# cvg/EMAP

Measured on AMD Instinct MI355X. Metric: ray-samples/sec (UDF MLP + composite), higher is better.
Workload: dtype f16x3 (split-fp16 MFMA, 3 passes, fp32 accumulate)

## Files before the change

### emap_amd/csrc/emap_common.h

```cpp
#pragma once
#include <hip/hip_runtime.h>
#include <stdint.h>
#include <stdio.h>
#include "../../include/emap_hip.h"


namespace emap {
constexpr float F16X3_WS = 8192.0f;
constexpr float F16_LO_SCALE = 2048.0f;

void set_error(const char* fmt, ...);
int check_launch(const char* what);

inline bool attr_needed(uint64_t& mask) {
    int d = 0;
    if (hipGetDevice(&d) != hipSuccess || d < 0 || d > 63) return true;
    if (mask & (1ull << d)) return false;
    mask |= 1ull << d;
    return true;
}
inline int raise_lds_limit(uint64_t& mask, const void* fn, int bytes = 160 * 1024) {
    if (attr_needed(mask) && hipFuncSetAttribute(fn, hipFuncAttributeMaxDynamicSharedMemorySize, bytes) != hipSuccess) {
        set_error("hipFuncSetAttribute(MaxDynamicSharedMemorySize) failed");
        return EMAP_E_LAUNCH;
    }
    return EMAP_OK;
}

constexpr int FRAG_BYTES = 1024;
constexpr int PE_KS = 2;

struct LayerDesc {
    int32_t pe_ks;
    int32_t h_ks;
    int32_t n_pairs;
    int32_t out_dim;
    int32_t in_prev;
    int32_t frag_off;
    int32_t act;
    int32_t pad;
};

struct NetLayout {
    int32_t H, n_lin, skip_l, multires, d0, nparts, udf_type, n_chunks;
    float scale;
    int32_t total_frags;
    int32_t bias_off_bytes, rowscale_off_bytes, frag_off_bytes;
    int32_t is_f16;
    int32_t mx_fwd;
    int32_t mx_bwd;
    int32_t has_rev, t_total_frags, t_frag_off_bytes, wlast_off_bytes;
    int32_t t_off[EMAP_MAX_LIN], tpe_off[EMAP_MAX_LIN];
    int32_t r32_frag_off_bytes, r32_t_frag_off_bytes;
    int32_t sweep_mx, swm_off_bytes, swm_units;
    int32_t wgrad_lo;
    int32_t swm_unit[EMAP_MAX_LIN], swm_t_unit[EMAP_MAX_LIN];
    LayerDesc layer[EMAP_MAX_LIN];
};
constexpr int SWM_UNIT_BYTES = 6656;
__host__ __device__ inline int t_hidden_frags(const NetLayout& L, int l) { return ((L.layer[l].in_prev + 31) / 32) * (L.H / 32) * 2 * L.nparts; }
__host__ __device__ inline int t_pe_frags(const NetLayout& L) { return 2 * (L.H / 32) * 2 * L.nparts; }
__host__ __device__ inline int swm_fwd_units(const NetLayout& L, int l) { return L.layer[l].n_pairs * (L.H / 128); }
__host__ __device__ inline int swm_rev_units(const NetLayout& L, int l) { return ((L.layer[l].in_prev + 31) / 32) * (L.H / 128); }

__host__ __device__ inline bool r32_t_mixed(const NetLayout& L) { return L.mx_bwd && L.is_f16 && L.nparts == 2 && L.H == 256; }
__host__ __device__ inline bool r32_mixed(const NetLayout& L) { return L.mx_fwd && r32_t_mixed(L); }
#define EMAP_PE_HI6_E8M0 125u
#define EMAP_PE_LO6_E8M0 124u
__host__ __device__ inline uint32_t mx6_scale_bits(float m) {
    const float mm = fmaxf(m, 7.8886090522101181e-31f ) * 1.0666667f;
    uint32_t b;
    __builtin_memcpy(&b, &mm, 4);
    return (b & 0x7f800000u) - (2u << 23);
}

int build_layout(const EmapNetConfig* cfg, int prec, NetLayout* L);
inline size_t layout_bytes(const NetLayout& L) {
    const size_t base = (size_t)L.r32_t_frag_off_bytes + (size_t)L.t_total_frags * FRAG_BYTES;
    return L.sweep_mx ? (size_t)L.swm_off_bytes + (size_t)L.swm_units * SWM_UNIT_BYTES : base;
}

int launch_pack(const NetLayout& L, const float* const* g, const float* const* v, const float* const* b,
                void* packed, hipStream_t st);

struct PointSource {
    const float* x;
    const float* rays_o;
// ... 201 lines not shown
```

### emap_amd/csrc/udf_mlp_vjp.inc

```
#pragma once

__device__ __forceinline__ void asm_gload4(uint32_t& dst, int voff, const char* sbase) {
    asm volatile("s_nop 4\n\tglobal_load_dword %0, %1, %2" : "=v"(dst) : "v"(voff), "s"(sbase) : "memory");
}
template <int N>
__device__ __forceinline__ void asm_wait_unit(u32x4& a, u32x4& b, u32x4& c, u32x4& d, u32x2& e, u32x2& f, u32x2& g, u32x2& h, uint32_t& i) {
    asm volatile("s_waitcnt vmcnt(%c9)" : "+v"(a), "+v"(b), "+v"(c), "+v"(d), "+v"(e), "+v"(f), "+v"(g), "+v"(h), "+v"(i) : "i"(N) : "memory");
}


struct VjpArgs {
    MlpArgs m;
    const float* d_udf;
    const float* d_grad;
    char* stash_a;
    char* stash_z;
    char* stash_s;
    const uint32_t* absmax;
    float* ldot;
    VjpLayout V;
    int32_t tile0;
    const char* swm;
    int32_t swm_unit[EMAP_MAX_LIN], swm_t_unit[EMAP_MAX_LIN];
};

template <int H, int MODE, int NW, bool SMX_ = false>
__global__ __launch_bounds__(NW * 64, NW == 8 ? 1 : 2) void udf_mlp_vjp_kernel(const VjpArgs va) {
    using T = typename Prec<MODE>::T;
    using V8 = typename Prec<MODE>::V;
    const MlpArgs& a = va.m;
    constexpr int NPART = Prec<MODE>::NPART;
    constexpr bool SCALED = (NPART == 2);
    constexpr float LO_SCALE = (MODE == EMAP_PREC_F16X3) ? F16_LO_SCALE : 1.0f;
    constexpr int NCT = 4;
    constexpr int NKS = H / 32;
    constexpr int NPAIR = H / 32;
    constexpr int NFR = 2 * NPART;
    constexpr int PD = 2;
    constexpr int PPW = NPAIR / NW;
    constexpr int KQ = NKS / NW;
    static_assert(PPW == 1 && PPW * NW == NPAIR && KQ * NW == NKS && NW >= 4, "waves per workgroup");
    constexpr bool SMX = SMX_ && MODE == EMAP_PREC_F16X3 && H == 256;
    constexpr int NSLAB = vjp_slab_planes(MODE == EMAP_PREC_F16X3, SMX);
    constexpr bool SLABLO = NSLAB > 4;
    typedef uint32_t u32x8 __attribute__((ext_vector_type(8)));

    extern __shared__ __attribute__((aligned(16))) char smem[];
    constexpr int XB = NKS * NCT * NPART * FRAG_BYTES;
    constexpr int PB = PE_KS * NCT * NPART * FRAG_BYTES;
    constexpr bool PP = (NW == 8);
    char* const xb0 = smem;
    char* const xb1 = smem + (PP ? XB : 0);
    char* pebuf = smem + (PP ? 2 : 1) * XB;
    float* red = reinterpret_cast<float*>(PP ? smem + 2 * XB + PB : smem);
    int cur = 0;

    const int tid = threadIdx.x;
    const int lane = tid & 63;
    const int wave = __builtin_amdgcn_readfirstlane(tid >> 6);
    const int g = lane >> 4;
    const int j = lane & 15;
    const int wvoff = lane * 16;
    const char* wbase = uniform_ptr(a.frags);
    const char* tbase = uniform_ptr(a.tfrags);
    const int n_hidden = a.n_lin - 1;
    const char* xr = xb0 + lane * 16;
    const int xm_lane = g * (NCT * NPART * FRAG_BYTES) + FRAG_BYTES;
    const char* xmr = xb0 + xm_lane;
    const char* per = pebuf + lane * 16;
    const int p0 = wave * PPW;
    V8 sel[2];
#pragma unroll
    for (int h = 0; h < 2; ++h)
#pragma unroll
        for (int e = 0; e < 8; ++e) sel[h][e] = ((j >> 2) == g && e == 4 * h + (j & 3)) ? (T)1.0f : (T)0.0f;
    char* const slab = va.stash_s + (size_t)blockIdx.x * ((size_t)va.V.s_slab_kb * 1024);
    const float Kscale = vjp_scale_from(va.absmax);

    clock_stamp(a.clk, 2);
    V8 hd[PD][NFR];
    auto load_head = [&](const char* wb) __attribute__((always_inline)) {
#pragma unroll
        for (int sp = 0; sp < PD; ++sp)
#pragma unroll
            for (int f = 0; f < NFR; ++f) {
                typedef const V8 __attribute__((address_space(1))) * gptr_t;
                hd[sp][f] = *(gptr_t)(uintptr_t)(wb + (sp * NFR + f) * FRAG_BYTES + wvoff);
            }
    };
    u32x2 hd6r[4];
    uint32_t hasc = 0;
    auto load_head_mx = [&](const char* wbh, const char* wm) __attribute__((always_inline)) {
        typedef const V8 __attribute__((address_space(1))) * gptr_t;
        typedef const u32x2 __attribute__((address_space(1))) * g2_t;
        typedef const uint32_t __attribute__((address_space(1))) * g1_t;
#pragma unroll
        for (int sp = 0; sp < PD; ++sp)
#pragma unroll
            for (int t = 0; t < 2; ++t) hd[sp][t] = *(gptr_t)(uintptr_t)(wbh + (sp * NFR + 2 * t) * FRAG_BYTES + wvoff);
#pragma unroll
        for (int t = 0; t < 2; ++t)
#pragma unroll
            for (int pt = 0; pt < 2; ++pt) {
                hd[t][2 + pt] = *(gptr_t)(uintptr_t)(wm + (2 * t + pt) * 1024 + wvoff);
                hd6r[2 * t + pt] = *(g2_t)(uintptr_t)(wm + 4096 + (2 * t + pt) * 512 + lane * 8);
            }
        hasc = *(g1_t)(uintptr_t)(wm + 6144 + lane * 4);
    };
    auto head_after_fwd = [&](int l) __attribute__((always_inline)) {
        int ln = l + 1;
        while (ln < n_hidden && p0 >= a.layer[ln].n_pairs) ++ln;
        const LayerDesc Ln = a.layer[ln < n_hidden ? ln : a.n_lin - 1];
        if constexpr (SMX) {
            if (ln >= n_hidden) return;
            if (!Ln.pe_ks) {
                load_head_mx(wbase + (size_t)(Ln.frag_off + p0 * Ln.h_ks * NFR) * FRAG_BYTES,
                             va.swm + (size_t)(va.swm_unit[ln] + p0 * (NKS / 4)) * SWM_UNIT_BYTES);
                return;
            }
        }
        const int first = (ln < n_hidden) ? p0 * (Ln.pe_ks + Ln.h_ks) : Ln.pe_ks + KQ * wave;
        load_head(wbase + (size_t)(Ln.frag_off + first * NFR) * FRAG_BYTES);
    };
    auto head_after_bwd = [&](int b, int tile) __attribute__((always_inline)) {
        int bn = b - 1;
        while (bn >= 1 && p0 >= a.layer[bn - 1].n_pairs) --bn;
        if (bn >= 1) {
            if constexpr (SMX) load_head_mx(tbase + (size_t)(a.t_off[bn] + p0 * NKS * NFR) * FRAG_BYTES,
                                            va.swm + (size_t)(va.swm_t_unit[bn] + p0 * (NKS / 4)) * SWM_UNIT_BYTES);
            else load_head(tbase + (size_t)(a.t_off[bn] + p0 * NKS * NFR) * FRAG_BYTES);
        }
        else if (tile + (int)gridDim.x < a.n_tiles) head_after_fwd(-1);
    };
    if ((int)blockIdx.x < a.n_tiles) head_after_fwd(-1);
    for (int i = tid * 16; i < (PP ? 2 : 1) * XB; i += NW * 64 * 16) *reinterpret_cast<f32x4*>(smem + i) = f32x4{0.f, 0.f, 0.f, 0.f};
    __syncthreads();
    for (int tile = blockIdx.x; tile < a.n_tiles; tile += gridDim.x) {
        const long long pbase = ((long long)va.tile0 + tile) * VJP_PT;
        char* const sa = va.stash_a + (size_t)tile * ((size_t)va.V.a_tile_kb * 1024);
        char* const sz = va.stash_z + (size_t)tile * ((size_t)va.V.z_tile_kb * 1024);
        constexpr bool LO_STASH = (NPART == 2) && !SMX;
        const bool stash_lo = LO_STASH && va.V.lo_a_delta != 0;
        auto stash_store = [&](char* level_pair, const V8 (&x)[4], int n_rt) __attribute__((always_inline)) {
            const f32x4 z4 = {0.f, 0.f, 0.f, 0.f};
#pragma unroll
            for (int h = 0; h < 2; ++h) {
                if (h < n_rt) {
                    f32x4 d[4];
#pragma unroll
                    for (int ct = 0; ct < 4; ++ct) d[ct] = mfma16(x[ct], sel[h], z4);
#pragma unroll
                    for (int ks = 0; ks < 2; ++ks) {
                        V8 v;
#pragma unroll
                        for (int e = 0; e < 8; ++e) v[e] = (T)d[2 * ks + (e >> 2)][e & 3];
                        *reinterpret_cast<V8*>(level_pair + (h * 2 + ks) * 1024 + lane * 16) = v;
                    }
                }
            }
        };

        if (wave < NCT) {
            const int ct = wave;
            int gq = g;
            asm volatile("" : "+v"(gq));
            float xs[3], vd[3] = {0.f, 0.f, 0.f};
            long long pp = pbase + 16 * (ct & 1) + j;
            const bool valid = pp < a.P;
            if (!valid) pp = a.P - 1;
            load_point(a.src, pp, a.scale, xs);
            if (ct >= 2 && valid) {
                vd[0] = va.d_grad[3 * pp + 0] * Kscale;
                vd[1] = va.d_grad[3 * pp + 1] * Kscale;
                vd[2] = va.d_grad[3 * pp + 2] * Kscale;
            }
            V8 f[PE_KS][NPART];
#pragma unroll
            for (int q = 0; q < 8; ++q) {
                const PeAngle ang = pe_angle(xs, 8 * gq + q, a.multires);
                float v0, v1;
                if (ct < 2) {
                    pe_pair(ang, xs, a.multires, 0, v0, v1);
                } else {
                    const float vc = (ang.c == 0) ? vd[0] : ((ang.c == 1) ? vd[1] : vd[2]);
                    const bool r0 = ang.a == 3 * a.multires, r1 = ang.a == 3 * a.multires + 1;
                    v0 = ang.is_ang ? ang.f * ang.cs * vc : (r0 ? vd[0] : (r1 ? vd[2] : 0.0f));
                    v1 = ang.is_ang ? -ang.f * ang.sn * vc : (r0 ? vd[1] : 0.0f);
                }
                const T h0 = (T)v0, h1 = (T)v1;
                f[q >> 2][0][2 * (q & 3)] = h0;
                f[q >> 2][0][2 * (q & 3) + 1] = h1;
                if constexpr (NPART == 2) {
                    f[q >> 2][1][2 * (q & 3)] = (T)((v0 - (float)h0) * LO_SCALE);
                    f[q >> 2][1][2 * (q & 3) + 1] = (T)((v1 - (float)h1) * LO_SCALE);
                }
            }
#pragma unroll
            for (int sp = 0; sp < PE_KS; ++sp)
#pragma unroll
                for (int pt = 0; pt < NPART; ++pt)
                    *reinterpret_cast<V8*>(pebuf + ((sp * NCT + ct) * NPART + pt) * FRAG_BYTES + lane * 16) = f[sp][pt];
        }
        __syncthreads();
        if (wave >= NW - PE_KS) {
            const int sp = wave - (NW - PE_KS);
            V8 c4[NCT];
#pragma unroll
            for (int ct = 0; ct < NCT; ++ct) c4[ct] = *reinterpret_cast<const V8*>(per + ((sp * NCT + ct) * NPART + 0) * FRAG_BYTES);
            stash_store(sa + (size_t)va.V.a_off[0] * 1024 + (2 * sp) * 2048, c4, 2);
            if constexpr (LO_STASH) {
                if (stash_lo) {
#pragma unroll
                    for (int ct = 0; ct < NCT; ++ct) c4[ct] = *reinterpret_cast<const V8*>(per + ((sp * NCT + ct) * NPART + (NPART - 1)) * FRAG_BYTES);
                    stash_store(sa + va.V.lo_a_delta + (size_t)va.V.a_off[0] * 1024 + (2 * sp) * 2048, c4, 2);
                }
            }
        }

        f32x4 acc[2][NCT];
        f32x4 accx[SCALED ? 2 : 1][NCT];
        V8 o[NCT][NPART];
        const f32x4 zero4 = {0.f, 0.f, 0.f, 0.f};

        auto zval = [&](int t, int ct, int r) __attribute__((always_inline)) -> float {
            if constexpr (SCALED) return fmaf(accx[t][ct][r], 1.0f / LO_SCALE, acc[t][ct][r]);
            else return acc[t][ct][r];
        };

        auto k_run_p = [&](auto ns_c, auto npe_c, auto init_c, auto pre_c, const char* wb, int xs0, int pes0, const float* bp) __attribute__((always_inline)) {
            constexpr int NS = decltype(ns_c)::value;
            constexpr int NPE = decltype(npe_c)::value;
            constexpr bool INIT = decltype(init_c)::value;
            constexpr bool PRE = decltype(pre_c)::value;
            V8 af[PD + 1][NFR];
            auto load_a = [&](auto s_c) __attribute__((always_inline)) {
                constexpr int s = decltype(s_c)::value;
#pragma unroll
                for (int f = 0; f < NFR; ++f) asm_gload16(af[s % (PD + 1)][f], wvoff, wb + (s * NFR + f) * FRAG_BYTES);
            };
            if constexpr (PRE) {
#pragma unroll
                for (int sp = 0; sp < PD; ++sp)
#pragma unroll
                    for (int f = 0; f < NFR; ++f) af[sp][f] = hd[sp][f];
            } else static_for<PD>([&](auto i_c) __attribute__((always_inline)) { if constexpr (decltype(i_c)::value < NS) load_a(i_c); });
            f32x4 i0 = zero4, i1 = zero4;
            if constexpr (INIT) {
                i0 = *reinterpret_cast<const f32x4*>(bp);
                i1 = *reinterpret_cast<const f32x4*>(bp + 16);
            }
            const char* xq = xr + xs0 * (NCT * NPART * FRAG_BYTES);
            const char* pq = per + pes0 * (NCT * NPART * FRAG_BYTES);
            V8 bh[NCT], bl[NCT];
            static_for<NS>([&](auto s_c) __attribute__((always_inline)) {
                constexpr int s = decltype(s_c)::value;
                constexpr int sa_ = s % (PD + 1);
                if constexpr (s == 0 && INIT) asm volatile("" : "+v"(i0), "+v"(i1));
                if constexpr (s + PD < NS) load_a(std::integral_constant<int, s + PD>{});
                constexpr bool is_pe = s < NPE;
                constexpr int sb = is_pe ? s : s - NPE;
#pragma unroll
                for (int ct = 0; ct < NCT; ++ct) {
                    const char* base = is_pe ? pq : xq;
                    bh[ct] = *reinterpret_cast<const V8*>(base + ((sb * NCT + ct) * NPART + 0) * FRAG_BYTES);
                    bl[ct] = *reinterpret_cast<const V8*>(base + ((sb * NCT + ct) * NPART + (NPART - 1)) * FRAG_BYTES);
                }
                {
                    constexpr int younger = ((s + PD < NS) ? PD : (NS - 1 - s)) * NFR;
#pragma unroll
                    for (int f = 0; f < NFR; f += 2) asm_wait_vm<younger>(af[sa_][f], af[sa_][f + 1]);
                }
                if constexpr (s == 0) {
#pragma unroll
                    for (int c2 = 0; c2 < NCT; ++c2) {
                        acc[0][c2] = (c2 < 2) ? i0 : zero4;
                        acc[1][c2] = (c2 < 2) ? i1 : zero4;
                        if constexpr (SCALED) { accx[0][c2] = zero4; accx[1][c2] = zero4; }
                    }
                }
                if constexpr (NPART == 1) {
#pragma unroll
                    for (int ct = 0; ct < NCT; ++ct) {
                        acc[0][ct] = mfma16(af[sa_][0], bh[ct], acc[0][ct]);
                        acc[1][ct] = mfma16(af[sa_][1], bh[ct], acc[1][ct]);
                    }
                } else {
#pragma unroll
                    for (int ct = 0; ct < NCT; ++ct) {
                        if constexpr (SCALED) { accx[0][ct] = mfma16(af[sa_][0], bl[ct], accx[0][ct]); accx[1][ct] = mfma16(af[sa_][2], bl[ct], accx[1][ct]); }
                        else { acc[0][ct] = mfma16(af[sa_][0], bl[ct], acc[0][ct]); acc[1][ct] = mfma16(af[sa_][2], bl[ct], acc[1][ct]); }
                    }
#pragma unroll
                    for (int ct = 0; ct < NCT; ++ct) {
                        acc[0][ct] = mfma16(af[sa_][0], bh[ct], acc[0][ct]);
                        acc[1][ct] = mfma16(af[sa_][2], bh[ct], acc[1][ct]);
                    }
#pragma unroll
// ... 149 lines not shown
                            const auto s02 = __builtin_amdgcn_permlane32_swap(x0, x2, false, false);
                            const auto s13 = __builtin_amdgcn_permlane32_swap(x1, x3, false, false);
                            const auto w01 = __builtin_amdgcn_permlane16_swap(s02[0], s13[0], false, false);
                            const auto w23 = __builtin_amdgcn_permlane16_swap(s02[1], s13[1], false, false);
                            blk[pt][0 * 4 + d] = w01[0]; blk[pt][1 * 4 + d] = w01[1]; blk[pt][2 * 4 + d] = w23[0]; blk[pt][3 * 4 + d] = w23[1];
                        }
                    auto block_max = [&](const u32x16& v) __attribute__((always_inline)) -> float {
                        uint32_t mb = 0;
#pragma unroll
                        for (int q = 0; q < 16; ++q)
                            asm("v_pk_maximum3_f16 %0, %1, %2, %2 neg_lo:[0,0,1] neg_hi:[0,0,1]" : "=v"(mb) : "v"(mb), "v"(v[q]));
                        const h2 m = __builtin_bit_cast(h2, mb);
                        return fmaxf((float)m[0], (float)m[1]);
                    };
                    const uint32_t sbh = mx6_scale_bits(block_max(blk[0])), sbl = mx6_scale_bits(block_max(blk[1]));
                    const u32x6 qh = __builtin_amdgcn_cvt_scalef32_pk32_fp6_f16(__builtin_bit_cast(f16x32, blk[0]), __builtin_bit_cast(float, sbh));
                    const u32x6 ql = __builtin_amdgcn_cvt_scalef32_pk32_fp6_f16(__builtin_bit_cast(f16x32, blk[1]), __builtin_bit_cast(float, sbl));
                    char* const dst = xbuf + ((p0 * NCT + g) * NPART + 1) * FRAG_BYTES;
                    *reinterpret_cast<u32x4*>(dst + j * 16) = u32x4{qh[0], qh[1], qh[2], qh[3]};
                    *reinterpret_cast<u32x4*>(dst + 256 + j * 16) = u32x4{ql[0], ql[1], ql[2], ql[3]};
                    *reinterpret_cast<u32x2*>(dst + 512 + j * 8) = u32x2{qh[4], qh[5]};
                    *reinterpret_cast<u32x2*>(dst + 640 + j * 8) = u32x2{ql[4], ql[5]};
                    *reinterpret_cast<uint32_t*>(dst + 768 + j * 4) = (sbh >> 23) | ((((sbl >> 23) - 11u) & 0xffu) << 8);
                }
            }
            __syncthreads();
            if constexpr (PP) { cur ^= 1; xr = (cur ? xb1 : xb0) + lane * 16; xmr = (cur ? xb1 : xb0) + xm_lane; }
        };
        using yes_t = std::true_type;
        using no_t = std::false_type;
        u32x4 sgv[4];
        auto load_slab = [&](const char* src) __attribute__((always_inline)) {
            const char* sb = uniform_ptr(src);
            static_for<4>([&](auto c_c) __attribute__((always_inline)) {
                constexpr int c = decltype(c_c)::value;
                asm_gload16_sc1<c * 1024>(sgv[c], wvoff, sb);
            });
        };
        auto wait_slab = [&]() __attribute__((always_inline)) {
            asm volatile("s_waitcnt vmcnt(0)" : "+v"(sgv[0]), "+v"(sgv[1]), "+v"(sgv[2]), "+v"(sgv[3]) : : "memory");
        };

        for (int l = 0; l < n_hidden; ++l) {
            const LayerDesc L = a.layer[l];
            const int kind = (L.h_ks == 0) ? KIND_FIRST : (L.pe_ks ? KIND_SKIP : KIND_NORMAL);
            const int p = p0;
            if (p < L.n_pairs) {
                const float* bp = a.bias + l * H + 32 * p + 4 * g;
                const int ns = L.pe_ks + L.h_ks;
                const char* wb = wbase + (size_t)(L.frag_off + p * ns * NFR) * FRAG_BYTES;
                if constexpr (SMX) {
                    const char* wm = va.swm + (size_t)(va.swm_unit[l] + p * (NKS / 4)) * SWM_UNIT_BYTES;
                    if (kind == KIND_NORMAL) k_run_mx(std::integral_constant<int, 1>{}, std::integral_constant<int, NKS / 4>{}, yes_t{}, 0, wb, wm, bp);
                    else if (kind == KIND_SKIP) {
                        k_run_p(std::integral_constant<int, PE_KS>{}, std::integral_constant<int, PE_KS>{}, yes_t{}, yes_t{}, wb, 0, 0, bp);
                        k_run_mx(std::integral_constant<int, 2>{}, std::integral_constant<int, NKS / 4>{}, no_t{}, 0, wb + (size_t)PE_KS * NFR * FRAG_BYTES, wm, bp);
                    } else k_run_p(std::integral_constant<int, PE_KS>{}, std::integral_constant<int, PE_KS>{}, yes_t{}, yes_t{}, wb, 0, 0, bp);
                } else {
                if (kind == KIND_NORMAL) k_run_p(std::integral_constant<int, NKS>{}, std::integral_constant<int, 0>{}, yes_t{}, yes_t{}, wb, 0, 0, bp);
                else if (kind == KIND_SKIP) k_run_p(std::integral_constant<int, PE_KS + NKS>{}, std::integral_constant<int, PE_KS>{}, yes_t{}, yes_t{}, wb, 0, 0, bp);
                else k_run_p(std::integral_constant<int, PE_KS>{}, std::integral_constant<int, PE_KS>{}, yes_t{}, yes_t{}, wb, 0, 0, bp);
                }
                head_after_fwd(l);
                uint32_t bk[SLABLO ? 24 : 16];
                static_for<8>([&](auto q_c) __attribute__((always_inline)) {
                    constexpr int q = decltype(q_c)::value, t = q >> 2, r = q & 3;
                    float a0, s0, a1, s1;
                    softplus_sig_fast(zval(t, 0, r), a0, s0);
                    softplus_sig_fast(zval(t, 1, r), a1, s1);
                    const float t0 = s0 * zval(t, 2, r), t1 = s1 * zval(t, 3, r);
                    put1(0, 4 * t + r, a0);
                    put1(1, 4 * t + r, a1);
                    typedef T T2 __attribute__((ext_vector_type(2)));
                    const T2 ap2 = {put1(2, 4 * t + r, t0), put1(3, 4 * t + r, t1)};
                    bk[2 * q] = __builtin_bit_cast(uint32_t, ap2);
                    bk[2 * q + 1] = __builtin_bit_cast(uint32_t, __builtin_amdgcn_cvt_pknorm_u16(s0, s1));
                    if constexpr (SLABLO) {
                        const T2 lo2 = {(T)((t0 - (float)ap2[0]) * LO_SCALE), (T)((t1 - (float)ap2[1]) * LO_SCALE)};
                        bk[16 + q] = __builtin_bit_cast(uint32_t, lo2);
                    }
                });
                {
                    const V8 xh[4] = {o[0][0], o[1][0], o[2][0], o[3][0]};
                    stash_store(sa + (size_t)va.V.a_off[l + 1] * 1024 + (2 * p) * 2048, xh, 2);
                }
                if constexpr (LO_STASH) {
                    if (stash_lo) {
                        const V8 xl[4] = {o[0][NPART - 1], o[1][NPART - 1], o[2][NPART - 1], o[3][NPART - 1]};
                        stash_store(sa + va.V.lo_a_delta + (size_t)va.V.a_off[l + 1] * 1024 + (2 * p) * 2048, xl, 2);
                    }
                }
                u32x4* dst = reinterpret_cast<u32x4*>(slab + ((size_t)(l * NPAIR + p) * NSLAB) * 1024 + lane * 16);
#pragma unroll
                for (int c = 0; c < NSLAB; ++c) dst[c * 64] = u32x4{bk[4 * c], bk[4 * c + 1], bk[4 * c + 2], bk[4 * c + 3]};
            }
            publish(L.n_pairs);
        }

        float hpart[NCT];
        {
            const LayerDesc L = a.layer[a.n_lin - 1];
            const char* wb = wbase + (size_t)(L.frag_off + (L.pe_ks + KQ * wave) * NFR) * FRAG_BYTES;
            if constexpr (SMX) {
#pragma unroll
                for (int ct = 0; ct < NCT; ++ct) hpart[ct] = 0.f;
                if (wave < NKS / 4) {
                    k_run_mx(std::integral_constant<int, 0>{}, std::integral_constant<int, 1>{}, no_t{}, wave, wbase + (size_t)L.frag_off * FRAG_BYTES,
                             va.swm + (size_t)va.swm_unit[a.n_lin - 1] * SWM_UNIT_BYTES, nullptr);
#pragma unroll
                    for (int ct = 0; ct < NCT; ++ct) hpart[ct] = zval(0, ct, 0);
                }
            } else {
            k_run_p(std::integral_constant<int, KQ>{}, std::integral_constant<int, 0>{}, no_t{}, yes_t{}, wb, KQ * wave, 0, nullptr);
#pragma unroll
            for (int ct = 0; ct < NCT; ++ct) hpart[ct] = zval(0, ct, 0);
            }
            if (L.pe_ks && wave < PE_KS) {
                const char* wp = wbase + (size_t)(L.frag_off + wave * NFR) * FRAG_BYTES;
                k_run(std::integral_constant<int, 1>{}, std::integral_constant<int, 1>{}, no_t{}, wp, 0, wave, nullptr);
#pragma unroll
                for (int ct = 0; ct < NCT; ++ct) hpart[ct] += zval(0, ct, 0);
            }
            head_after_bwd(a.n_lin - 1, tile);
            if constexpr (!PP) __syncthreads();
            if (g == 0) {
#pragma unroll
                for (int ct = 0; ct < NCT; ++ct) red[(wave * NCT + ct) * 16 + j] = hpart[ct];
            }
        }
        __syncthreads();
        float seed[NCT];
        {
            float hs[NCT];
#pragma unroll
            for (int ct = 0; ct < NCT; ++ct) {
                float v = 0.f;
#pragma unroll
                for (int w = 0; w < NW; ++w) v += red[(w * NCT + ct) * 16 + j];
                hs[ct] = v;
            }
            const float b_last = a.bias[(a.n_lin - 1) * H];
            const float inv_scale = 1.0f / a.scale;
            bool bad = false;
#pragma unroll
            for (int c = 0; c < 2; ++c) {
                const long long pp = pbase + 16 * c + j;
                const float h = hs[c] + b_last, hp = hs[c + 2];
                float u1, u2;
                if (a.udf_type == EMAP_UDF_ABS) { u1 = (h > 0.f) ? 1.f : ((h < 0.f) ? -1.f : 0.f); u2 = 0.f; }
                else if (a.udf_type == EMAP_UDF_SQUARE) { u1 = 2.f * h; u2 = 2.f; }
                else { u1 = 1.f; u2 = 0.f; }
                const bool valid = pp < a.P;
                const float du = valid ? va.d_udf[pp] * Kscale : 0.f;
                seed[c] = valid ? fmaf(du * inv_scale, u1, u2 * hp) : 0.f;
                seed[c + 2] = valid ? u1 : 0.f;
                bad |= valid && !(fabsf(h) + fabsf(hp) <= 3.0e38f);
            }
            if (wave == 0 && g == 0) flag_nonfinite(a.err, bad);
            if (wave == 0 && g == 0) {
                float d = seed[0] * hs[0] + seed[1] * hs[1] + seed[2] * hs[2] + seed[3] * hs[3];
#pragma unroll
                for (int off = 8; off > 0; off >>= 1) d += __shfl_xor(d, off);
                if (j == 0) va.ldot[va.tile0 + tile] = d;
            }
        }
        if (wave == 0) {
            V8 xs[4];
#pragma unroll
            for (int ct = 0; ct < NCT; ++ct) {
                const T hi = (T)seed[ct];
#pragma unroll
                for (int e = 0; e < 8; ++e) xs[ct][e] = (T)0.0f;
                xs[ct][0] = (g == 0) ? hi : (T)0.0f;
                xs[ct][1] = (g == 0) ? (T)(seed[ct] - (float)hi) : (T)0.0f;
            }
            stash_store(sz + (size_t)va.V.z_off[a.n_lin - 1] * 1024, xs, 1);
            if constexpr (LO_STASH) {
                if (stash_lo) {
#pragma unroll
                    for (int ct = 0; ct < NCT; ++ct)
#pragma unroll
                        for (int e = 0; e < 8; ++e) xs[ct][e] = (T)0.0f;
                    stash_store(sz + va.V.lo_z_delta + (size_t)va.V.z_off[a.n_lin - 1] * 1024, xs, 1);
                }
            }
        }

        for (int b = a.n_lin - 1; b >= 1; --b) {
            const int lz = b - 1;
            const int p = p0;
            if (p < a.layer[lz].n_pairs) {
                load_slab(slab + ((size_t)(lz * NPAIR + p) * NSLAB) * 1024);
                if (b == a.n_lin - 1) {
                    const f32x4 w0 = *reinterpret_cast<const f32x4*>(a.wlast + 32 * p + 4 * g);
                    const f32x4 w1 = *reinterpret_cast<const f32x4*>(a.wlast + 32 * p + 16 + 4 * g);
#pragma unroll
                    for (int ct = 0; ct < NCT; ++ct) {
                        acc[0][ct] = w0 * seed[ct];
                        acc[1][ct] = w1 * seed[ct];
                        if constexpr (SCALED) { accx[0][ct] = zero4; accx[1][ct] = zero4; }
                    }
                } else {
                    const char* wb = tbase + (size_t)(a.t_off[b] + p * NKS * NFR) * FRAG_BYTES;
                    if constexpr (SMX) k_run_mx(std::integral_constant<int, 0>{}, std::integral_constant<int, NKS / 4>{}, yes_t{}, 0, wb,
                                                va.swm + (size_t)(va.swm_t_unit[b] + p * (NKS / 4)) * SWM_UNIT_BYTES, nullptr);
                    else k_run_p(std::integral_constant<int, NKS>{}, std::integral_constant<int, 0>{}, no_t{}, yes_t{}, wb, 0, 0, nullptr);
                }
                wait_slab();
                u32x4 aplo[2];
                if constexpr (SLABLO) {
                    const char* lp = uniform_ptr(slab + ((size_t)(lz * NPAIR + p) * NSLAB + 4) * 1024);
                    asm_gload16_sc1<0>(aplo[0], wvoff, lp);
                    asm_gload16_sc1<1024>(aplo[1], wvoff, lp);
                    asm volatile("s_waitcnt vmcnt(0)" : "+v"(aplo[0]), "+v"(aplo[1]) : : "memory");
                }
                if (b != a.n_lin - 1) head_after_bwd(b, tile);
                static_for<8>([&](auto q_c) __attribute__((always_inline)) {
                    constexpr int q = decltype(q_c)::value, t = q >> 2, r = q & 3;
                    typedef T T2 __attribute__((ext_vector_type(2)));
                    const uint32_t apk = sgv[q >> 1][2 * (q & 1)], spk = sgv[q >> 1][2 * (q & 1) + 1];
                    const T2 ap2 = __builtin_bit_cast(T2, apk);
                    float ap0 = (float)ap2[0], ap1 = (float)ap2[1];
                    if constexpr (SLABLO) {
                        const uint32_t lok = aplo[q >> 2][q & 3];
                        const T2 lo2 = __builtin_bit_cast(T2, lok);
                        ap0 = fmaf((float)lo2[0], 1.0f / LO_SCALE, ap0);
                        ap1 = fmaf((float)lo2[1], 1.0f / LO_SCALE, ap1);
                    }
                    const float s0 = (float)(spk & 0xffffu) * (1.0f / 65535.0f);
                    const float s1 = (float)(spk >> 16) * (1.0f / 65535.0f);
                    const float av0 = zval(t, 0, r), av1 = zval(t, 1, r), at0 = zval(t, 2, r), at1 = zval(t, 3, r);
                    const float zb0 = fmaf(100.0f * (1.0f - s0) * ap0, at0, s0 * av0);
                    const float zb1 = fmaf(100.0f * (1.0f - s1) * ap1, at1, s1 * av1);
                    put1(0, 4 * t + r, zb0);
                    put1(1, 4 * t + r, zb1);
                    put1(2, 4 * t + r, s0 * at0);
                    put1(3, 4 * t + r, s1 * at1);
                });
                {
                    const V8 xh[4] = {o[0][0], o[1][0], o[2][0], o[3][0]};
                    stash_store(sz + (size_t)va.V.z_off[lz] * 1024 + (2 * p) * 2048, xh, 2);
                }
                if constexpr (LO_STASH) {
                    if (stash_lo) {
                        const V8 xl[4] = {o[0][NPART - 1], o[1][NPART - 1], o[2][NPART - 1], o[3][NPART - 1]};
                        stash_store(sz + va.V.lo_z_delta + (size_t)va.V.z_off[lz] * 1024 + (2 * p) * 2048, xl, 2);
                    }
                }
            }
            if (b > 1) publish(a.layer[lz].n_pairs);
        }
        __syncthreads();
    }
    clock_stamp(a.clk, 3);
}

template <int H, int MODE, int NW, bool SMX_ = false>
static int launch_vjp_sweep_t(const NetLayout& L, const void* packed, const VjpSweep& s, hipStream_t st, int32_t* err) {
    constexpr int NPART = Prec<MODE>::NPART;
    VjpArgs va;
    memset(&va, 0, sizeof(va));
    va.m = fill_mlp_args(L, packed, L.frag_off_bytes, L.t_frag_off_bytes, s.src, s.P, err);
    va.m.n_tiles = s.n_tiles; va.tile0 = s.tile0;
    va.m.clk = prof_clk_here();
    va.d_udf = s.d_udf; va.d_grad = s.d_grad; va.stash_a = s.stash_a; va.stash_z = s.stash_z; va.stash_s = s.stash_s; va.absmax = s.absmax; va.ldot = s.ldot; va.V = *s.V;
    va.swm = static_cast<const char*>(packed) + L.swm_off_bytes;
    for (int l = 0; l < L.n_lin; ++l) { va.swm_unit[l] = L.swm_unit[l]; va.swm_t_unit[l] = L.swm_t_unit[l]; }
    const size_t lds = (NW == 8) ? (size_t)(2 * (H / 32) + PE_KS) * 4 * NPART * FRAG_BYTES + (size_t)NW * 4 * 16 * 4
                                 : (size_t)((H / 32) + PE_KS) * 4 * NPART * FRAG_BYTES;
    auto kern = udf_mlp_vjp_kernel<H, MODE, NW, SMX_>;
    static uint64_t attr_mask = 0;
    const int rc = raise_lds_limit(attr_mask, reinterpret_cast<const void*>(kern));
    if (rc) return rc;
    if (s.n_tiles <= 0) return EMAP_OK;
    hipLaunchKernelGGL(kern, dim3(s.grid < s.n_tiles ? s.grid : s.n_tiles), dim3(NW * 64), lds, st, va);
    return check_launch("udf_mlp_vjp");
}

template <int MODE>
int launch_vjp_sweep_mode(const NetLayout& L, const void* packed, const VjpSweep& s, hipStream_t st, int32_t* err) {
    if constexpr (MODE == EMAP_PREC_F16X3) {
        if (L.H == 256 && L.sweep_mx) return launch_vjp_sweep_t<256, MODE, 8, true>(L, packed, s, st, err);
    }
    if (L.H == 256) return launch_vjp_sweep_t<256, MODE, 8>(L, packed, s, st, err);
    if (L.H == 128) return launch_vjp_sweep_t<128, MODE, 4>(L, packed, s, st, err);
    set_error("no training-backward kernel for d_hidden=%d", L.H);
    return EMAP_E_INVALID;
}
```

### emap_amd/csrc/wgrad.hip

```cpp
#include "emap_common.h"
#include <string.h>

namespace emap {

typedef __bf16 bf16x8 __attribute__((ext_vector_type(8)));
typedef _Float16 f16x8 __attribute__((ext_vector_type(8)));
typedef float f32x4 __attribute__((ext_vector_type(4)));

__device__ __forceinline__ f32x4 mfma16w(const bf16x8& a, const bf16x8& b, const f32x4& c) { return __builtin_amdgcn_mfma_f32_16x16x32_bf16(a, b, c, 0, 0, 0); }
__device__ __forceinline__ f32x4 mfma16w(const f16x8& a, const f16x8& b, const f32x4& c) { return __builtin_amdgcn_mfma_f32_16x16x32_f16(a, b, c, 0, 0, 0); }

__global__ __launch_bounds__(256) void absmax_kernel(const float* du, const float* dg, long long P, uint32_t* out) {
    float mu = 0.f, mg = 0.f;
    for (long long i = (long long)blockIdx.x * 256 + threadIdx.x; i < P; i += (long long)gridDim.x * 256) {
        const float u = fabsf(du[i]);
        const float g = fmaxf(fmaxf(fabsf(dg[3 * i]), fabsf(dg[3 * i + 1])), fabsf(dg[3 * i + 2]));
        mu = (u < 3.0e38f) ? fmaxf(mu, u) : mu;
        mg = (g < 3.0e38f) ? fmaxf(mg, g) : mg;
    }
#pragma unroll
    for (int off = 32; off > 0; off >>= 1) { mu = fmaxf(mu, __shfl_xor(mu, off)); mg = fmaxf(mg, __shfl_xor(mg, off)); }
    if ((threadIdx.x & 63) == 0) {
        atomicMax(out, __builtin_bit_cast(uint32_t, mu));
        atomicMax(out + 1, __builtin_bit_cast(uint32_t, mg));
    }
}

struct WgradArgs {
    const char* stash_a;
    const char* stash_z;
    float* partial;
    int32_t n_tiles, n_jobs, a_tile_kb, z_tile_kb;
    int32_t accumulate;
    float scale;
    int32_t no_bias;
    WgradJob job[WGRAD_MAX_JOBS];
};

template <int CT>
__device__ __forceinline__ void wgrad_store(const WgradArgs& a, const WgradJob& J, int slice, int wave, int lane, f32x4 (&acc)[2][CT], float (&bsum)[2]) {
    float* pb = a.partial + J.part_off + (size_t)slice * 16 * J.a_ct * 256;
#pragma unroll
    for (int i = 0; i < 2; ++i) {
        const int rt = wave + 8 * i;
        if (rt < J.z_rt) {
#pragma unroll
            for (int c = 0; c < CT; ++c) {
                if (c < J.a_ct) {
                    f32x4* dst = reinterpret_cast<f32x4*>(pb + ((size_t)rt * J.a_ct + c) * 256 + lane * 4);
                    *dst = a.accumulate ? (*dst + acc[i][c] * a.scale) : acc[i][c] * a.scale;
                }
            }
        }
    }
    if (J.bias_off >= 0 && !a.no_bias) {
#pragma unroll
        for (int i = 0; i < 2; ++i) {
            float v = bsum[i] * a.scale;
            v += __shfl_xor(v, 16);
            v += __shfl_xor(v, 32);
            const int rt = wave + 8 * i;
            if (rt < J.z_rt && lane < 16) {
                float* dst = a.partial + J.bias_off + (size_t)slice * 256 + rt * 16 + lane;
                *dst = a.accumulate ? (*dst + v) : v;
            }
        }
    }
}

#ifndef EMAP_REDUCE_WAVES
#define EMAP_REDUCE_WAVES 4
#endif
#ifndef EMAP_WGRAD_DEPTH
#define EMAP_WGRAD_DEPTH 3
#endif
constexpr int WGRAD_DEPTH = EMAP_WGRAD_DEPTH;
__device__ __forceinline__ void wg_dma16(unsigned lds_dst, const char* gsrc) {
    unsigned keep;
    asm volatile("s_mov_b32 %0, m0\n\ts_mov_b32 m0, %2\n\ts_nop 0\n\tglobal_load_lds_dwordx4 %1, off\n\ts_mov_b32 m0, %0"
                 : "=&s"(keep) : "v"(gsrc), "s"(lds_dst) : "memory");
}

template <class V8, int NB>
__device__ __forceinline__ void wgrad_lds_run(const WgradArgs& a, const WgradJob& J, int slice, int wave, int lane, char* smem) {
    constexpr int CT = 4 * NB;
    constexpr int NA = (CT + 7) / 8;
    constexpr int NLD = NA + 2;
    constexpr int D = WGRAD_DEPTH, NST = D + 1;
    constexpr int STAGE = (CT + 16) * 1024;
    const int t0 = (int)(((long long)a.n_tiles * slice) / J.n_slices), t1 = (int)(((long long)a.n_tiles * (slice + 1)) / J.n_slices);
    const int nsteps = 2 * (t1 - t0);
    f32x4 acc[2][CT];
#pragma unroll
    for (int i = 0; i < 2; ++i)
#pragma unroll
        for (int c = 0; c < CT; ++c) acc[i][c] = f32x4{0.f, 0.f, 0.f, 0.f};
    float bsum[2] = {0.f, 0.f};
    if (nsteps > 0) {
        const size_t zts = (size_t)a.z_tile_kb * 1024, ats = (size_t)a.a_tile_kb * 1024;
        const char* zsrc = a.stash_z + (size_t)J.z_off * 1024 + lane * 16;
        const char* asrc = a.stash_a + (size_t)J.a_off * 1024 + lane * 16;
        const unsigned lds0 = (unsigned)(size_t)smem;
        int ca[NA], zr[2];
#pragma unroll
        for (int i = 0; i < NA; ++i) ca[i] = 8 * i + ((8 * i + 8 <= CT) ? wave : wave % (CT - 8 * i));
        zr[0] = wave < J.z_rt ? wave : J.z_rt - 1;
        zr[1] = wave + 8 < J.z_rt ? wave + 8 : J.z_rt - 1;
        auto issue = [&](int u) __attribute__((always_inline)) {
            const int uu = u < nsteps ? u : nsteps - 1;
            const int tile = t0 + (uu >> 1), sh = (uu & 1) * 1024;
            const unsigned st = lds0 + (unsigned)(u % NST) * STAGE;
#pragma unroll
            for (int i = 0; i < NA; ++i) {
                const int cs = ca[i] < J.a_ct ? ca[i] : J.a_ct - 1;
                wg_dma16(__builtin_amdgcn_readfirstlane(st + ca[i] * 1024), asrc + (size_t)tile * ats + cs * 2048 + sh);
            }
#pragma unroll
            for (int i = 0; i < 2; ++i)
                wg_dma16(__builtin_amdgcn_readfirstlane(st + (CT + zr[i]) * 1024), zsrc + (size_t)tile * zts + zr[i] * 2048 + sh);
        };
        for (int u = 0; u < D; ++u) issue(u);
        for (int u = 0; u < nsteps; ++u) {
            asm volatile("s_waitcnt vmcnt(%0)" :: "i"(NLD * (D - 1)) : "memory");
            __builtin_amdgcn_s_barrier();
            issue(u + D);
            const char* st = smem + (size_t)(u % NST) * STAGE + lane * 16;
            V8 z[2];
            z[0] = *reinterpret_cast<const V8*>(st + (CT + zr[0]) * 1024);
            z[1] = *reinterpret_cast<const V8*>(st + (CT + zr[1]) * 1024);
            {
                const float m = (u & 1) ? 0.0f : 1.0f;
#pragma unroll
                for (int i = 0; i < 2; ++i)
                    bsum[i] = fmaf(m, (((float)z[i][0] + (float)z[i][1]) + ((float)z[i][2] + (float)z[i][3])) +
                                      (((float)z[i][4] + (float)z[i][5]) + ((float)z[i][6] + (float)z[i][7])), bsum[i]);
            }
#pragma unroll
            for (int c = 0; c < CT; ++c) {
                const V8 af = *reinterpret_cast<const V8*>(st + c * 1024);
                acc[0][c] = mfma16w(z[0], af, acc[0][c]);
                acc[1][c] = mfma16w(z[1], af, acc[1][c]);
            }
        }
        asm volatile("s_waitcnt vmcnt(0)" ::: "memory");
    }
    wgrad_store<CT>(a, J, slice, wave, lane, acc, bsum);
}

#ifdef EMAP_WGRAD_TIMING
static __device__ long long emap_wg_times[1024 * 2];
#endif
template <class V8>
__global__ __launch_bounds__(512, 1) void wgrad_kernel(const WgradArgs a) {
    extern __shared__ __attribute__((aligned(16))) char wg_smem[];
#ifdef EMAP_WGRAD_TIMING
    const long long wg_t0 = __builtin_amdgcn_s_memrealtime();
#endif
    int ji = 0;
    while (ji + 1 < a.n_jobs && (int)blockIdx.x >= a.job[ji + 1].first_wg) ++ji;
    const WgradJob J = a.job[ji];
    const int slice = (int)blockIdx.x - J.first_wg;
    const int lane = threadIdx.x & 63;
    const int wave = __builtin_amdgcn_readfirstlane(threadIdx.x >> 6);
    const int nb = (J.a_ct + 3) >> 2;
    if (nb <= 1) wgrad_lds_run<V8, 1>(a, J, slice, wave, lane, wg_smem);
    else if (nb == 2) wgrad_lds_run<V8, 2>(a, J, slice, wave, lane, wg_smem);
    else if (nb == 3) wgrad_lds_run<V8, 3>(a, J, slice, wave, lane, wg_smem);
    else wgrad_lds_run<V8, 4>(a, J, slice, wave, lane, wg_smem);
#ifdef EMAP_WGRAD_TIMING
    if (threadIdx.x == 0 && blockIdx.x < 1024) { emap_wg_times[2 * blockIdx.x] = ji; emap_wg_times[2 * blockIdx.x + 1] = __builtin_amdgcn_s_memrealtime() - wg_t0; }
#endif
}

struct ReduceArgs {
    const float* partial;
    const uint32_t* absmax;
    const float* ldot;
    int32_t n_tiles;
    float grad_scale;
    int32_t accumulate;
    int32_t weight_norm;
    int32_t n_lin, H, d0, multires, skip_l;
    int32_t row_off[EMAP_MAX_LIN + 1];
    int32_t out_dim[EMAP_MAX_LIN], in_prev[EMAP_MAX_LIN], has_pe[EMAP_MAX_LIN];
    int32_t job_h[EMAP_MAX_LIN], job_pe[EMAP_MAX_LIN];
    WgradJob job[WGRAD_MAX_JOBS];
    const float* g[EMAP_MAX_LIN];
    const float* v[EMAP_MAX_LIN];
    float* dg[EMAP_MAX_LIN];
    float* dv[EMAP_MAX_LIN];
    float* db[EMAP_MAX_LIN];
};

__device__ __forceinline__ float wave_sum_f(float v) {
#pragma unroll
    for (int off = 32; off > 0; off >>= 1) v += __shfl_xor(v, off);
    return v;
}

constexpr int RED_WAVES = EMAP_REDUCE_WAVES;
static_assert(RED_WAVES >= 2 && RED_WAVES <= 16, "EMAP_REDUCE_WAVES: the cross-wave sum needs 2..16 waves (part[RED_WAVES - 1] in LDS)");
__global__ __launch_bounds__(RED_WAVES * 64) void wgrad_reduce_kernel(const ReduceArgs a) {
    __shared__ f32x4 part[RED_WAVES - 1][6][64];
    const int grp = blockIdx.x;
    const int wv = threadIdx.x >> 6;
    const int lane = threadIdx.x & 63;
    if (grp >= a.row_off[a.n_lin]) return;
    int l = 0;
    while (grp >= a.row_off[l + 1]) ++l;
    const int o0 = 4 * (grp - a.row_off[l]);
    const int out_dim = a.out_dim[l];
    const int in_prev = a.in_prev[l];
    const int n_in = in_prev + (a.has_pe[l] ? a.d0 : 0);
    const float inv_k = a.grad_scale / vjp_scale_from(a.absmax);
    const float mult = (l == a.skip_l) ? 0.70710678118654752440f : 1.0f;
    const int rt = o0 >> 4, mq = (o0 & 15) >> 2;
    const bool last = (l == a.n_lin - 1);
    constexpr int MAXC = 6;
    float dw[4][MAXC], vv[4][MAXC];
    float dot[4] = {0.f, 0.f, 0.f, 0.f}, nrm[4] = {0.f, 0.f, 0.f, 0.f};
    const float* src[MAXC];
    size_t str[MAXC];
// ... 237 lines not shown
```

Baseline: 118.1 million.

## Store activation stash in natural layout and transpose via LDS read_tr in wgrad

Drops the MFMA-based identity-matrix transpose that the forward/VJP pass used when writing activations and z-gradients to the stash, storing fragments directly in a swizzled layout instead. The weight-gradient kernel now reads the stage from LDS with ds_read_tr16_b64 transposing loads, with a shared header defining store, fetch and read offsets. The last-z level uses a compact half-width layout. This removes extra MFMA and conversion work from the forward path, but makes correctness depend on the offset maps agreeing across both kernels and adds two LDS reads per fragment.

```diff
diff --git a/emap_amd/csrc/emap_common.h b/emap_amd/csrc/emap_common.h
--- a/emap_amd/csrc/emap_common.h
+++ b/emap_amd/csrc/emap_common.h
@@ -3,6 +3,7 @@
 #include <stdint.h>
 #include <stdio.h>
 #include "../../include/emap_hip.h"
+#include "stash_maps.h"
 
 
 namespace emap {
diff --git a/emap_amd/csrc/stash_maps.h b/emap_amd/csrc/stash_maps.h
--- /dev/null
+++ b/emap_amd/csrc/stash_maps.h
@@ -0,0 +1,42 @@
+#pragma once
+
+#ifndef EMAP_HD
+#if defined(__HIPCC__) || defined(__CUDACC__)
+#define EMAP_HD __host__ __device__
+#else
+#define EMAP_HD
+#endif
+#endif
+
+namespace emap {
+namespace stash {
+
+enum Kind { PAIR = 0, LAST_Z = 1 };
+constexpr int FRAG = 1024;
+
+EMAP_HD constexpr int z_kind(int z_rt) { return z_rt == 1 ? LAST_Z : PAIR; }
+
+EMAP_HD constexpr int phi(int g, int e) { return 16 * (e >> 2) + 4 * g + (e & 3); }
+
+EMAP_HD constexpr int slot(int g, int j) { return 16 * g + (j ^ ((g & 1) << 3)); }
+
+EMAP_HD constexpr int store_bytes(int kind) { return kind == PAIR ? 16 : 8; }
+EMAP_HD constexpr int store_offset(int kind, int pair, int ct, int lane) {
+    return kind == PAIR ? pair * 4 * FRAG + ct * FRAG + 16 * slot(lane >> 4, lane & 15) : ct * (FRAG / 2) + 8 * lane;
+}
+
+EMAP_HD constexpr int fetch_frags(int kind, int rt) { return kind == PAIR ? (rt + 1) & ~1 : 1; }
+EMAP_HD constexpr int fetch_offset(int kind, int f, int ks) {
+    return kind == PAIR ? (f >> 1) * 4 * FRAG + ks * 2 * FRAG + (f & 1) * FRAG : ks * FRAG;
+}
+
+EMAP_HD constexpr int read_offset(int kind, int rt, int r, int lane) {
+    const int kg = lane >> 4, q = (lane >> 2) & 3, p = lane & 3, j = 4 * kg + q;
+    return kind == PAIR ? ((rt & ~1) + r) * FRAG + 16 * slot(p, j) + 8 * (rt & 1) : r * (FRAG / 2) + 8 * (16 * p + j);
+}
+
+struct Elem { int feature, ct, point; };
+EMAP_HD constexpr Elem read_elem(int rt, int ks, int r, int lane, int e) { return Elem{16 * rt + (lane & 15), 2 * ks + r, 4 * (lane >> 4) + e}; }
+
+}
+}
diff --git a/emap_amd/csrc/udf_mlp_vjp.inc b/emap_amd/csrc/udf_mlp_vjp.inc
--- a/emap_amd/csrc/udf_mlp_vjp.inc
+++ b/emap_amd/csrc/udf_mlp_vjp.inc
@@ -69,11 +69,6 @@
     const char* xmr = xb0 + xm_lane;
     const char* per = pebuf + lane * 16;
     const int p0 = wave * PPW;
-    V8 sel[2];
-#pragma unroll
-    for (int h = 0; h < 2; ++h)
-#pragma unroll
-        for (int e = 0; e < 8; ++e) sel[h][e] = ((j >> 2) == g && e == 4 * h + (j & 3)) ? (T)1.0f : (T)0.0f;
     char* const slab = va.stash_s + (size_t)blockIdx.x * ((size_t)va.V.s_slab_kb * 1024);
     const float Kscale = vjp_scale_from(va.absmax);
 
@@ -141,24 +136,18 @@
         char* const sz = va.stash_z + (size_t)tile * ((size_t)va.V.z_tile_kb * 1024);
         constexpr bool LO_STASH = (NPART == 2) && !SMX;
         const bool stash_lo = LO_STASH && va.V.lo_a_delta != 0;
-        auto stash_store = [&](char* level_pair, const V8 (&x)[4], int n_rt) __attribute__((always_inline)) {
-            const f32x4 z4 = {0.f, 0.f, 0.f, 0.f};
-#pragma unroll
-            for (int h = 0; h < 2; ++h) {
-                if (h < n_rt) {
-                    f32x4 d[4];
-#pragma unroll
-                    for (int ct = 0; ct < 4; ++ct) d[ct] = mfma16(x[ct], sel[h], z4);
-#pragma unroll
-                    for (int ks = 0; ks < 2; ++ks) {
-                        V8 v;
-#pragma unroll
-                        for (int e = 0; e < 8; ++e) v[e] = (T)d[2 * ks + (e >> 2)][e & 3];
-                        *reinterpret_cast<V8*>(level_pair + (h * 2 + ks) * 1024 + lane * 16) = v;
-                    }
-                }
-            }
-        };
+        auto stash_store = [&](char* level, auto kind_c, int pair, const V8 (&x)[4]) __attribute__((always_inline)) {
+            constexpr int kind = decltype(kind_c)::value;
+            char* const dst = level + pair * (4 * stash::FRAG) + stash::store_offset(kind, 0, 0, lane);
+#pragma unroll
+            for (int ct = 0; ct < 4; ++ct) {
+                constexpr int step = stash::store_offset(kind, 0, 1, 0) - stash::store_offset(kind, 0, 0, 0);
+                if constexpr (kind == stash::PAIR) *reinterpret_cast<V8*>(dst + ct * step) = x[ct];
+                else *reinterpret_cast<u32x2*>(dst + ct * step) = __builtin_bit_cast(u32x4, x[ct]).xy;
+            }
+        };
+        using pair_k = std::integral_constant<int, stash::PAIR>;
+        using lastz_k = std::integral_constant<int, stash::LAST_Z>;
 
         if (wave < NCT) {
             const int ct = wave;
@@ -207,12 +196,12 @@
             V8 c4[NCT];
 #pragma unroll
             for (int ct = 0; ct < NCT; ++ct) c4[ct] = *reinterpret_cast<const V8*>(per + ((sp * NCT + ct) * NPART + 0) * FRAG_BYTES);
-            stash_store(sa + (size_t)va.V.a_off[0] * 1024 + (2 * sp) * 2048, c4, 2);
+            stash_store(sa + (size_t)va.V.a_off[0] * 1024, pair_k{}, sp, c4);
             if constexpr (LO_STASH) {
                 if (stash_lo) {
 #pragma unroll
                     for (int ct = 0; ct < NCT; ++ct) c4[ct] = *reinterpret_cast<const V8*>(per + ((sp * NCT + ct) * NPART + (NPART - 1)) * FRAG_BYTES);
-                    stash_store(sa + va.V.lo_a_delta + (size_t)va.V.a_off[0] * 1024 + (2 * sp) * 2048, c4, 2);
+                    stash_store(sa + va.V.lo_a_delta + (size_t)va.V.a_off[0] * 1024, pair_k{}, sp, c4);
                 }
             }
         }
@@ -528,12 +517,12 @@
                 });
                 {
                     const V8 xh[4] = {o[0][0], o[1][0], o[2][0], o[3][0]};
-                    stash_store(sa + (size_t)va.V.a_off[l + 1] * 1024 + (2 * p) * 2048, xh, 2);
+                    stash_store(sa + (size_t)va.V.a_off[l + 1] * 1024, pair_k{}, p, xh);
                 }
                 if constexpr (LO_STASH) {
                     if (stash_lo) {
                         const V8 xl[4] = {o[0][NPART - 1], o[1][NPART - 1], o[2][NPART - 1], o[3][NPART - 1]};
-                        stash_store(sa + va.V.lo_a_delta + (size_t)va.V.a_off[l + 1] * 1024 + (2 * p) * 2048, xl, 2);
+                        stash_store(sa + va.V.lo_a_delta + (size_t)va.V.a_off[l + 1] * 1024, pair_k{}, p, xl);
                     }
                 }
                 u32x4* dst = reinterpret_cast<u32x4*>(slab + ((size_t)(l * NPAIR + p) * NSLAB) * 1024 + lane * 16);
@@ -620,14 +609,14 @@
                 xs[ct][0] = (g == 0) ? hi : (T)0.0f;
                 xs[ct][1] = (g == 0) ? (T)(seed[ct] - (float)hi) : (T)0.0f;
             }
-            stash_store(sz + (size_t)va.V.z_off[a.n_lin - 1] * 1024, xs, 1);
+            stash_store(sz + (size_t)va.V.z_off[a.n_lin - 1] * 1024, lastz_k{}, 0, xs);
             if constexpr (LO_STASH) {
                 if (stash_lo) {
 #pragma unroll
                     for (int ct = 0; ct < NCT; ++ct)
 #pragma unroll
                         for (int e = 0; e < 8; ++e) xs[ct][e] = (T)0.0f;
-                    stash_store(sz + va.V.lo_z_delta + (size_t)va.V.z_off[a.n_lin - 1] * 1024, xs, 1);
+                    stash_store(sz + va.V.lo_z_delta + (size_t)va.V.z_off[a.n_lin - 1] * 1024, lastz_k{}, 0, xs);
                 }
             }
         }
@@ -685,12 +674,12 @@
                 });
                 {
                     const V8 xh[4] = {o[0][0], o[1][0], o[2][0], o[3][0]};
-                    stash_store(sz + (size_t)va.V.z_off[lz] * 1024 + (2 * p) * 2048, xh, 2);
+                    stash_store(sz + (size_t)va.V.z_off[lz] * 1024, pair_k{}, p, xh);
                 }
                 if constexpr (LO_STASH) {
                     if (stash_lo) {
                         const V8 xl[4] = {o[0][NPART - 1], o[1][NPART - 1], o[2][NPART - 1], o[3][NPART - 1]};
-                        stash_store(sz + va.V.lo_z_delta + (size_t)va.V.z_off[lz] * 1024 + (2 * p) * 2048, xl, 2);
+                        stash_store(sz + va.V.lo_z_delta + (size_t)va.V.z_off[lz] * 1024, pair_k{}, p, xl);
                     }
                 }
             }
diff --git a/emap_amd/csrc/wgrad.hip b/emap_amd/csrc/wgrad.hip
--- a/emap_amd/csrc/wgrad.hip
+++ b/emap_amd/csrc/wgrad.hip
@@ -81,6 +81,15 @@
                  : "=&s"(keep) : "v"(gsrc), "s"(lds_dst) : "memory");
 }
 
+template <class V8>
+__device__ __forceinline__ V8 wg_read_tr(unsigned lds0, unsigned lds1) {
+    typedef short s16x4 __attribute__((ext_vector_type(4)));
+    typedef short s16x8 __attribute__((ext_vector_type(8)));
+    typedef __attribute__((address_space(3))) s16x4* lds_t;
+    const s16x4 lo = __builtin_amdgcn_ds_read_tr16_b64_v4i16((lds_t)lds0), hi = __builtin_amdgcn_ds_read_tr16_b64_v4i16((lds_t)lds1);
+    return __builtin_bit_cast(V8, __builtin_shufflevector(lo, hi, 0, 1, 2, 3, 4, 5, 6, 7));
+}
+
 template <class V8, int NB>
 __device__ __forceinline__ void wgrad_lds_run(const WgradArgs& a, const WgradJob& J, int slice, int wave, int lane, char* smem) {
     constexpr int CT = 4 * NB;
@@ -101,33 +110,42 @@
         const char* zsrc = a.stash_z + (size_t)J.z_off * 1024 + lane * 16;
         const char* asrc = a.stash_a + (size_t)J.a_off * 1024 + lane * 16;
         const unsigned lds0 = (unsigned)(size_t)smem;
-        int ca[NA], zr[2];
+        const int zkind = stash::z_kind(J.z_rt);
+        const int a_nf = stash::fetch_frags(stash::PAIR, J.a_ct), z_nf = stash::fetch_frags(zkind, J.z_rt);
+        int ca[NA], zf[2], zr[2];
+        unsigned zo[2][2];
 #pragma unroll
         for (int i = 0; i < NA; ++i) ca[i] = 8 * i + ((8 * i + 8 <= CT) ? wave : wave % (CT - 8 * i));
-        zr[0] = wave < J.z_rt ? wave : J.z_rt - 1;
-        zr[1] = wave + 8 < J.z_rt ? wave + 8 : J.z_rt - 1;
+#pragma unroll
+        for (int i = 0; i < 2; ++i) {
+            zf[i] = wave + 8 * i < z_nf ? wave + 8 * i : z_nf - 1;
+            zr[i] = wave + 8 * i < J.z_rt ? wave + 8 * i : J.z_rt - 1;
+#pragma unroll
+            for (int r = 0; r < 2; ++r) zo[i][r] = (unsigned)(CT * 1024 + stash::read_offset(zkind, zr[i], r, lane));
+        }
+        const unsigned ao = (unsigned)stash::read_offset(stash::PAIR, 0, 0, lane);
         auto issue = [&](int u) __attribute__((always_inline)) {
             const int uu = u < nsteps ? u : nsteps - 1;
-            const int tile = t0 + (uu >> 1), sh = (uu & 1) * 1024;
+            const int tile = t0 + (uu >> 1), ks = uu & 1;
             const unsigned st = lds0 + (unsigned)(u % NST) * STAGE;
 #pragma unroll
             for (int i = 0; i < NA; ++i) {
-                const int cs = ca[i] < J.a_ct ? ca[i] : J.a_ct - 1;
-                wg_dma16(__builtin_amdgcn_readfirstlane(st + ca[i] * 1024), asrc + (size_t)tile * ats + cs * 2048 + sh);
+                const int cs = ca[i] < a_nf ? ca[i] : a_nf - 1;
+                wg_dma16(__builtin_amdgcn_readfirstlane(st + ca[i] * 1024), asrc + (size_t)tile * ats + stash::fetch_offset(stash::PAIR, cs, ks));
             }
 #pragma unroll
             for (int i = 0; i < 2; ++i)
-                wg_dma16(__builtin_amdgcn_readfirstlane(st + (CT + zr[i]) * 1024), zsrc + (size_t)tile * zts + zr[i] * 2048 + sh);
+                wg_dma16(__builtin_amdgcn_readfirstlane(st + (CT + zf[i]) * 1024), zsrc + (size_t)tile * zts + stash::fetch_offset(zkind, zf[i], ks));
         };
         for (int u = 0; u < D; ++u) issue(u);
         for (int u = 0; u < nsteps; ++u) {
             asm volatile("s_waitcnt vmcnt(%0)" :: "i"(NLD * (D - 1)) : "memory");
             __builtin_amdgcn_s_barrier();
             issue(u + D);
-            const char* st = smem + (size_t)(u % NST) * STAGE + lane * 16;
+            const unsigned st = lds0 + (unsigned)(u % NST) * STAGE;
             V8 z[2];
-            z[0] = *reinterpret_cast<const V8*>(st + (CT + zr[0]) * 1024);
-            z[1] = *reinterpret_cast<const V8*>(st + (CT + zr[1]) * 1024);
+            z[0] = wg_read_tr<V8>(st + zo[0][0], st + zo[0][1]);
+            z[1] = wg_read_tr<V8>(st + zo[1][0], st + zo[1][1]);
             {
                 const float m = (u & 1) ? 0.0f : 1.0f;
 #pragma unroll
@@ -135,9 +153,10 @@
                     bsum[i] = fmaf(m, (((float)z[i][0] + (float)z[i][1]) + ((float)z[i][2] + (float)z[i][3])) +
                                       (((float)z[i][4] + (float)z[i][5]) + ((float)z[i][6] + (float)z[i][7])), bsum[i]);
             }
+            const unsigned sa = st + ao;
 #pragma unroll
             for (int c = 0; c < CT; ++c) {
-                const V8 af = *reinterpret_cast<const V8*>(st + c * 1024);
+                const V8 af = wg_read_tr<V8>(sa + (unsigned)stash::read_offset(stash::PAIR, c, 0, 0), sa + (unsigned)stash::read_offset(stash::PAIR, c, 1, 0));
                 acc[0][c] = mfma16w(z[0], af, acc[0][c]);
                 acc[1][c] = mfma16w(z[1], af, acc[1][c]);
             }
```

Result: no change. 118.0 million (-0.1%).
